# ccuchengwei/LongReadSelfCorrect

Measured on AMD Instinct MI355X. Metric: corrected Mbases/s (whole node), higher is better.
Workload: dtype int64

## Files before the change

longreadselfcorrect_amd/csrc/capi_correct.cpp:

```cpp
#include "capi_internal.h"

using namespace lrsc;

struct lrsc::CorrectScratch {
    DevBuf<ReadPlan> d_plan;
    DevBuf<uint32_t> d_pieces;
    DevBuf<uint8_t> d_codes_out;
    DevBuf<uint64_t> d_dst_off;
    DevBuf<char> d_dst;
    DevBuf<double> d_freqs;
    DpStage stage;
    DevBuf<WpReadWork> d_work;
    DevBuf<WpRead> d_reads;
    DevBuf<WpSlot> d_slots;
    DevBuf<uint64_t> d_sz;
    DevBuf<uint32_t> d_key, d_key_tmp, d_list, d_list_tmp;
    DevBuf<uint32_t> d_small;
    DevBuf<WpDpItem> d_items, d_items2, d_items3;
    DevBuf<DevCounters> d_ctr2;
    hipEvent_t ev_side_t0 = nullptr, ev_side_t1 = nullptr;
    DevBuf<WpRequest> d_req;
    DevBuf<uint8_t> d_prep, d_lane, d_lane_side, d_lane_wide;
    DevBuf<uint32_t> d_wide_list;
    DevBuf<uint32_t> d_sort9;
// ... 510 lines not shown
    for(unsigned m = 1; m < 34; ++m)
        if(hist[m]) std::fprintf(stderr, " %u:%.2f%%(%.1f%%)", m, 100.0 * hist[m] / n_range, 100.0 * wsteps[m] / std::max(tot, 1ull));
    const uint32_t qs[] = {n_range / 2, n_range / 10, n_range / 100, n_range / 1000, n_range / 10000};
    std::fprintf(stderr, "; leaf-steps at the median / top 10%% / 1%% / 0.1%% / 0.01%%: %u %u %u %u %u\n", hs[ord[qs[0]]].leaf_steps, hs[ord[qs[1]]].leaf_steps,
                 hs[ord[qs[2]]].leaf_steps, hs[ord[qs[3]]].leaf_steps, hs[ord[qs[4]]].leaf_steps);
    return LRSC_OK;
}

void WpFlow::print_round(const Round& R) const
{
    std::fprintf(stderr, "[lrsc] wp reads [%u, %u) round %u: %u entries, %u DP requests (%llu strings), arenas q %.1f MB prep %.1f MB path %.1f MB, %llu walks escalated so far\n",
                 r0, r1, R.index, R.n_ent, R.n_items, (unsigned long long)sc.stage.n_strings, R.tot[0] / 1048576.0, R.tot[1] / 1048576.0, R.tot[2] / 1048576.0,
                 (unsigned long long)n_escalated);
    const unsigned long long* g = R.begin_stats;
    if(tn.wp_begin_sort)
        std::fprintf(stderr, "[lrsc] wp reads [%u, %u) round %u: wp_begin %llu interval lists, %llu entries, every list sorted (LRSC_WP_BEGIN_SORT)\n",
                     r0, r1, R.index, g[0], g[2] + g[3]);
    else
        std::fprintf(stderr, "[lrsc] wp reads [%u, %u) round %u: wp_begin %llu interval lists, %llu with a repeated code (%.1f%%); entries %llu in the lists without one, %llu in those with one\n",
                     r0, r1, R.index, g[0], g[1], 100.0 * g[1] / std::max(g[0], 1ull), g[2], g[3]);
}

int WpFlow::print_extension_profile()
{
    unsigned long long prs[32];
    HIP_TRY(hipStreamSynchronize(ctx->stream));
    HIP_TRY(hipStreamSynchronize(sc.side));
    HIP_TRY(hipMemcpy(prs, sc.d_prof.p, sizeof(prs), hipMemcpyDeviceToHost));
    for(int part = 0; part < 2; ++part) {
        const unsigned long long* pr = prs + 16 * part;
        if(pr[10] == 0) continue;
        const double all = (double)pr[10], st = (double)std::max<unsigned long long>(pr[11], 1);
        std::fprintf(stderr, "[lrsc] wp extension kernel (%s), lane wall ticks: %.3g total, %.0f per step over %.3g steps; extendLeaves %.1f%% (refine %.1f%%, attempToExtend %.1f%% of which "
                             "getFMIndexExtensions %.1f%%), PrunedBySeedSupport %.1f%%, materialise+commit %.1f%%, isTerminated %.1f%%, refill %.1f%%, finish %.1f%%; single-leaf fast steps %.1f%% of the steps in %.1f%% of the ticks\n",
                     part ? "long-gap walks, one per wavefront" : "bulk and later rounds",
                     all, all / st, st, 100 * pr[0] / all, 100 * pr[1] / all, 100 * pr[2] / all, 100 * pr[3] / all, 100 * pr[4] / all, 100 * pr[5] / all, 100 * pr[6] / all,
                     100 * pr[8] / all, 100 * pr[9] / all, 100 * pr[12] / st, 100 * pr[7] / all);
    }
    return LRSC_OK;
}

int WpFlow::gather_results(lrsc_read_result* res, uint64_t* piece_off, uint64_t piece_cap, char* out, uint64_t out_cap,
                           uint64_t* n_pieces_out, uint64_t* out_used)
{
    std::vector<WpRead> ro(n);
    COPY_TRY(ctx, ro.data(), sc.d_reads.p, (size_t)n * sizeof(WpRead), hipMemcpyDeviceToHost);
    std::vector<uint32_t> pieces(std::max<uint64_t>(piece_total, 1));
    if(piece_total) COPY_TRY(ctx, pieces.data(), sc.d_pieces.p, (size_t)piece_total * sizeof(uint32_t), hipMemcpyDeviceToHost);
    std::vector<uint64_t> dst_off(n + 1, 0);
    uint64_t n_pieces = 0;
    for(uint32_t r = 0; r < n; ++r) {
        const WpRead& o = ro[r];
        int status = skipped[r];
        if(o.error == LRSC_WALK_ERR_GEOMETRY) status = LRSC_READ_GEOMETRY;
        else if(o.error == LRSC_WALK_ERR_CODE) status = LRSC_READ_INTERNAL;
        else if(o.error == LRSC_WALK_ERR_DP) status = LRSC_READ_DP_LIMIT;
        else if(o.error == LRSC_WALK_ERR_OUTPUT) status = LRSC_READ_OUTPUT_LIMIT;
        else if(o.error != 0) status = LRSC_READ_FRONTIER_LIMIT;
        lrsc_read_result& R = res[r];
        if(status != LRSC_READ_OK) {
            std::memset(&R, 0, sizeof(R));
            R.piece_first = n_pieces;
            R.status = status;
            dst_off[r + 1] = dst_off[r];
            continue;
        }
        R.merge = (int32_t)o.merge; R.n_pieces = o.n_pieces; R.piece_first = n_pieces;
        R.total_reads_len = (int64_t)(off[r + 1] - off[r]); R.corrected_len = o.c[1]; R.total_seed_num = seed_count[r]; R.total_walk_num = o.c[3];
        R.high_error_num = o.c[4]; R.exceed_depth_num = o.c[5]; R.exceed_leave_num = o.c[6]; R.fm_num = o.c[7];
// ... 64 lines not shown
```

longreadselfcorrect_amd/csrc/walk_device.h:

```cpp
#pragma once
#include <hip/hip_runtime.h>

#include "extend.h"
#include "introsort_emul.h"
#include "rank_device.h"

#ifndef LRSC_WALK_NOINLINE
#define LRSC_WALK_NOINLINE __noinline__
#endif
#ifndef LRSC_WALK_FN
#define LRSC_WALK_FN __device__
#endif

namespace lrsc {

constexpr uint64_t kNoKey = ~0ull;

template <bool WIDE>
LRSC_WALK_FN __forceinline__ void prepare_offset(const FmIndexDev& fm, const StrandC<typename Lay<WIDE>::pos_t>& sf,
                                               const StrandC<typename Lay<WIDE>::pos_t>& sr, const uint32_t* __restrict__ mtab,
                                               const uint8_t* __restrict__ q, uint32_t i, uint32_t Lq, uint32_t trg0,
                                               uint32_t seedk, uint32_t mink, SortItem* it9f, SortItem* it9r, uint8_t* flags5,
                                               typename Lay<WIDE>::pos_t* term, uint32_t& n_rank, uint32_t& n_blk)
{
    using P = typename Lay<WIDE>::pos_t;
    const bool want_term = i >= trg0 && i + mink <= Lq;
    uint32_t kmax = 0;
    if(i + 5 <= Lq) kmax = 5;
    if(i + seedk <= Lq) kmax = seedk;
    if(want_term) kmax = mink > kmax ? mink : kmax;
    WalkState<P> st = walk_init<P>();
    for(uint32_t s = 0; s < kmax;) {
        const uint32_t next_emit = s < 5 ? 5u : s < seedk ? seedk : mink;
        bool jumped = false;
        if(next_emit <= kmax) {
            WalkState<P> ts = walk_init<P>();
            const uint32_t tk = table_start<WIDE>(fm, [&](uint32_t t) { return (uint32_t)q[i + t]; }, next_emit, ts);
            if(tk == next_emit) { n_rank += st.n_rank; n_blk += st.n_blk; st = ts; st.n_rank = 0; st.n_blk = 0; s = tk; jumped = true; }
        }
        if(!jumped) { st = walk_step<WIDE>(sf, sr, q[i + s], 1u << 30, st, mtab); ++s; }
        if(st.size == 5) flags5[i] = (uint8_t)((st.fwd.lo <= st.fwd.hi ? 1 : 0) | (st.rvc.lo <= st.rvc.hi ? 2 : 0));
        if(st.size == seedk) {
            uint32_t code = 0;
            for(uint32_t t = 0; t < seedk; ++t) code = (code << 2) | q[i + t];
// ... 309 lines not shown
            const uint32_t back = U - 1 - t;
            return back < 32 ? (uint32_t)(slo >> (2 * back)) & 3u : (uint32_t)(shi >> (2 * (back - 32))) & 3u;
        };
        bool fb = false, rb = false;
        uint32_t t1 = 1;
        {
            WalkState<P> ts = walk_init<P>();
            const uint32_t tk = table_start<WIDE>(*fm, [&](uint32_t t) { return 3u - sc(U - 1 - t); }, Lw, ts);
            if(tk != 0) {
                f = ts.rvc; r = ts.fwd; fb = ts.rvc_broken; rb = ts.fwd_broken; t1 = tk;
            } else {
                f = init_interval<P>(sR, sc(U - 1));
                r = init_interval<P>(sF, 3u - sc(U - 1));
                n_rank += 2;
            }
        }
        for(uint32_t t = t1; t < Lw; ++t) {
            if(fb && rb) break;
            const uint32_t c = sc(U - 1 - t);
            if(!fb) { f = upd(sR, c, f); fb = f.lo > f.hi; }
            if(!rb) { r = upd(sF, 3u - c, r); rb = r.lo > r.hi; }
            if(fb && rb) break;
        }
    }
    LRSC_WALK_FN __forceinline__ void select_next(uint64_t slo, uint64_t shi, uint32_t U, uint32_t t, IvT<P>& f, IvT<P>& r)
    {
        const uint32_t back = U - 1 - t;
        const uint32_t b = back < 32 ? (uint32_t)(slo >> (2 * back)) & 3u : (uint32_t)(shi >> (2 * (back - 32))) & 3u;
        f = upd(sR, b, f);
        r = upd(sF, 3u - b, r);
    }
    LRSC_WALK_FN LRSC_WALK_NOINLINE uint64_t SelectFreqsOfrange(uint64_t LowerBound, uint64_t UpperBound, Leaf<P>* leaves, uint32_t n)
    {
        int tempmaxfmfreqs = 0;
        const uint32_t U = (uint32_t)UpperBound, Lw = (uint32_t)LowerBound;
        for(uint32_t j = 0; j < n; ++j) {
            Leaf<P>& lf = leaves[j];
            IvT<P> f, r;
            select_first(lf.suf_lo, lf.suf_hi, U, Lw, f, r);
            lf.tflo = f.lo; lf.tfhi = f.hi; lf.trlo = r.lo; lf.trhi = r.hi;
            lf.tmpFreq = (int)(isize(f.lo, f.hi) + isize(r.lo, r.hi));
            if(lf.tmpFreq > tempmaxfmfreqs) tempmaxfmfreqs = lf.tmpFreq;
        }
        if(tempmaxfmfreqs - (int)freqsOfKmerSize[LowerBound] < 5) return LowerBound;

        for(uint64_t i = 1; i <= UpperBound - LowerBound; i++) {
            tempmaxfmfreqs = 0;
            for(uint32_t j = 0; j < n; ++j) {
                Leaf<P>& lf = leaves[j];
                IvT<P> f{lf.tflo, lf.tfhi}, r{lf.trlo, lf.trhi};
                select_next(lf.suf_lo, lf.suf_hi, U, (uint32_t)(UpperBound - LowerBound - i), f, r);
                lf.tflo = f.lo; lf.tfhi = f.hi; lf.trlo = r.lo; lf.trhi = r.hi;
                lf.tmpFreq = (int)(isize(f.lo, f.hi) + isize(r.lo, r.hi));
                if(lf.tmpFreq > tempmaxfmfreqs) tempmaxfmfreqs = lf.tmpFreq;
            }
            if(tempmaxfmfreqs - (int)freqsOfKmerSize[LowerBound + i] < 5) return LowerBound + i;
        }
        return UpperBound;
    }
    LRSC_WALK_FN __forceinline__ uint64_t SelectFreqsOfrange1(uint64_t LowerBound, uint64_t UpperBound, uint64_t slo, uint64_t shi)
    {
        const uint32_t U = (uint32_t)UpperBound, Lw = (uint32_t)LowerBound;
        IvT<P> f, r;
        select_first(slo, shi, U, Lw, f, r);
        int freq = (int)(isize(f.lo, f.hi) + isize(r.lo, r.hi));
        int tempmaxfmfreqs = freq > 0 ? freq : 0;
// ... 96 lines not shown
    }

    LRSC_WALK_FN void attempToExtend()
    {
        double minimumErrorRate = 1;
        for(uint32_t i = 0; i < n_cur; i += 4) {
            double e[4];
#pragma unroll
            for(uint32_t j = 0; j < 4; ++j) e[j] = cur[i + j < n_cur ? i + j : i].localErr;
#pragma unroll
            for(uint32_t j = 0; j < 4; ++j) if(i + j < n_cur && e[j] < minimumErrorRate) minimumErrorRate = e[j];
        }
        uint32_t w = 0;
        for(uint32_t i = 0; i < n_cur; ++i) {
            const double errorRateDiff = cur[i].localErr - minimumErrorRate;
            if((errorRateDiff > 0.05 && currentLength > localK / 2) || (errorRateDiff > 0.1 && currentLength > 15)) {
                free_leaf_slots(cur[i]);
                continue;
            }
            if(w != i) leaf_move(&cur[w], &cur[i]);
            ++w;
        }
        n_cur = w;

        n_highfreq = 0;
        const int highfreqThreshold = PBcoverage > 60 ? (int)((uint64_t)(PBcoverage / 60) * 3) : 3;
        for(uint32_t i = 0; i < n_cur; ++i) {
            const Leaf<P> par = cur[i];
            Ext ext[4];
            uint32_t mask = 0;
            int count = 0;
            while(count < 2) {
                if(count == 1 && !(par.localErr == minimumErrorRate && n_cur > 1)) break;
                uint64_t tc;
                const uint64_t tg = tick();
                mask = getFMIndexExtensions_v(par.flo, par.fhi, par.rlo, par.rhi, par.tailLetterCount, par.suf_lo, ext, tc);
                tock(3, tg);
                if(mask != 0) break;
                min_SA_threshold--;
                count++;
            }
            min_SA_threshold += (uint64_t)count;
            if(mask == 0) continue;
            for(uint32_t b = 0; b < 4; ++b) {
                if(!(mask & (1u << b))) continue;
                if(n_nxt >= max_children()) { error = LRSC_WALK_ERR_CHILDREN; return; }
                const Leaf<P> ch = make_child(par, i, b, ext[b]);
                if(ch.kmerFrequency > highfreqThreshold) n_highfreq++;
                nxt[n_nxt++] = ch;
            }
        }
    }
    LRSC_WALK_FN __forceinline__ Leaf<P> make_child(const Leaf<P>& par, uint32_t i, uint32_t b, const Ext& e) const
    {
        Leaf<P> ch = par;
        ch.flo = e.f.lo; ch.fhi = e.f.hi; ch.rlo = e.r.lo; ch.rhi = e.r.hi;
        ch.kmerFrequency = e.freq;
        ch.currOverlapLen++;
        ch.queryOverlapLen++;
        if(par.tailLetter == b) ch.tailLetterCount = par.tailLetterCount + 1;
        else { ch.tailLetter = b; ch.tailLetterCount = 1; }
        suf_push(ch, b);
        ch.parent = (uint16_t)i;
        ch.ext = (uint8_t)b;
        ch.alive = 1;
        return ch;
    }

    LRSC_WALK_FN void extendLeaves()
    {
        n_nxt = 0;
        uint64_t t = tick();
        if(currentKmerSize > maxOverlap) refineSAInterval(cur, n_cur, maxOverlap);
        tock(1, t);
        t = tick();
        attempToExtend();
        tock(2, t);
        if(error) return;
        if(n_nxt == 0) {
            const uint64_t LowerBound = (currentKmerSize - 2) > minOverlap ? (currentKmerSize - 2) : minOverlap;
            const uint64_t ReduceSize = SelectFreqsOfrange(LowerBound, currentKmerSize, cur, n_cur);
            refineSAInterval(cur, n_cur, ReduceSize);
            attempToExtend();
            if(error) return;
            if(n_nxt == 0) {
                min_SA_threshold--;
                attempToExtend();
                min_SA_threshold++;
                if(error) return;
            }
        }
        if(n_nxt != 0) {
            currentLength++;
            currentKmerSize++;
            if(isInsufficientFreqs(n_highfreq, n_nxt)) {
                const uint64_t LowerBound = (currentKmerSize - 2) > minOverlap ? (currentKmerSize - 2) : minOverlap;
                const uint64_t ReduceSize = SelectFreqsOfrange(LowerBound, currentKmerSize, nxt, n_nxt);
                refineSAInterval(nxt, n_nxt, ReduceSize);
            }
        }
    }

    LRSC_WALK_FN LRSC_WALK_NOINLINE bool isSupportedByNewSeed(Leaf<P>& nd, uint64_t smallSeedIdx, uint64_t largeSeedIdx)
    {
        return seed_support_core(nd, smallSeedIdx, largeSeedIdx);
    }
    LRSC_WALK_FN __forceinline__ bool seed_support_core(Leaf<P>& nd, uint64_t smallSeedIdx, uint64_t largeSeedIdx)
    {
        const uint64_t seedIdxOffset = nd.lastOverlapLen < currentLength - seedSize ? (uint64_t)seedSize : currentLength - nd.lastOverlapLen;
        const uint64_t cand = nd.lastSeedIdx + seedIdxOffset;
        const uint64_t startSeedIdx = smallSeedIdx > cand ? smallSeedIdx : cand;
        bool isNewSeedFound = false;
        const bool fv = nd.flo <= nd.fhi, rv = nd.rlo <= nd.rhi;
        const uint32_t mask9 = seedSize >= 16 ? 0xFFFFFFFFu : ((1u << (2 * seedSize)) - 1u);
        const uint32_t code9 = (uint32_t)nd.suf_lo & mask9;
        const uint32_t hb = (code9 ^ (code9 >> 9)) & 255u;
        uint32_t jf = fv ? head9f[hb] : 0xFFFFu;
        uint32_t jr = rv ? head9r[hb] : 0xFFFFu;
        auto advance = [&](uint32_t j, const SortItem* it, const uint16_t* nx) -> uint32_t {
            while(j != 0xFFFFu && it[j].pad != code9) j = nx[j];
            return j;
        };
        jf = advance(jf, it9f, next9f);
        jr = advance(jr, it9r, next9r);
        int minIdxDiff = 10000;
        const uint64_t currSeedIdx = currentLength - seedSize;
        while(jf != 0xFFFFu || jr != 0xFFFFu) {
            const uint64_t vf = jf != 0xFFFFu ? it9f[jf].val : 0, vr = jr != 0xFFFFu ? it9r[jr].val : 0;
            if(fv && jf != 0xFFFFu && vf >= startSeedIdx && vf <= largeSeedIdx) {
                const int d = abs((int)vf - (int)currSeedIdx);
// ... 31 lines not shown
        double currErrorRate = unmatchedLen / totalLen;
        nd.globalErr = currErrorRate;
        const uint32_t totalsize = nd.hist_size + 1;
        nd.hist_size = totalsize;
        if(totalsize >= localK) {
            const double old = parent_ring[(totalsize - localK) % 100];
            currErrorRate = (currErrorRate * totalLen - old * (totalLen - localK)) / localK;
        }
        nd.localErr = currErrorRate;
        return currErrorRate;
    }

    template <bool INLINE>
    LRSC_WALK_FN __forceinline__ void prune_leaf(Leaf<P>& leaf, const double* pring, uint64_t currSeedIdx, uint64_t smallSeedIdx, uint64_t largeSeedIdx)
    {
        bool isNewSeedFound = false;
        if(currentLength - leaf.lastOverlapLen > seedSize || currentLength - leaf.lastOverlapLen <= 1) {
            const uint64_t preSeedIdx = leaf.lastSeedIdx;
            isNewSeedFound = INLINE ? seed_support_core(leaf, smallSeedIdx, largeSeedIdx) : isSupportedByNewSeed(leaf, smallSeedIdx, largeSeedIdx);
            if(isNewSeedFound) {
                if(currSeedIdx + (uint64_t)(int64_t)leaf.lastSeedIdxOffset - preSeedIdx > seedSize)
                    leaf.numRedeemSeed += (seedSize - 1) * PacBioErrorRate;
                leaf.lastSeedIdxOffset = (int)leaf.lastSeedIdx - (int)currSeedIdx;
            } else {
                const uint64_t v = currSeedIdx + (uint64_t)(int64_t)leaf.lastSeedIdxOffset - leaf.lastSeedIdx;
                if(v % seedSize == 1) leaf.numOfErrors++;
                else if(v > (uint64_t)seedSize - 1) leaf.numRedeemSeed += 1 - PacBioErrorRate;
            }
        } else
            leaf.numRedeemSeed += 1 - PacBioErrorRate;
        const double currErrorRate = computeErrorRate(leaf, pring);
        if(currErrorRate > errorRate) leaf.alive = 0;
    }
    LRSC_WALK_FN void PrunedBySeedSupport()
    {
        const uint64_t currSeedIdx = currentLength - seedSize;
        const uint64_t indelOffset = seedSize + maxIndelSize;
        const uint64_t smallSeedIdx = currSeedIdx <= indelOffset ? 0 : currSeedIdx - indelOffset;
        const uint64_t largeSeedIdx = (currSeedIdx + indelOffset) >= (Lq - seedSize) ? (Lq - seedSize) : currSeedIdx + indelOffset;
        alive_lo = 0; alive_hi = 0; has_child = 0;
        if constexpr(BIG) { bits_clear_all(this->alive_bits, n_nxt); bits_clear_all(this->child_bits, n_cur); }
        for(uint32_t c = 0; c < n_nxt; ++c) {
            Leaf<P> leaf = nxt[c];
            prune_leaf<true>(leaf, rings + (uint64_t)leaf.ring * 100, currSeedIdx, smallSeedIdx, largeSeedIdx);
            nxt[c] = leaf;
            if constexpr(BIG) { if(leaf.alive) { bits_set(this->alive_bits, c); bits_set(this->child_bits, leaf.parent); } }
            else if(leaf.alive) { if(c < 64) alive_lo |= 1ull << c; else alive_hi |= 1ull << (c - 64); has_child |= 1u << leaf.parent; }
        }
    }

    LRSC_WALK_FN LRSC_WALK_NOINLINE void terminated_leaf(Leaf<P>& lf, const uint32_t* pw, uint32_t plen, int extra)
    {
        const int hit = term_scan(lf);
        if(hit < 0) return;
        if(lf.res_first == -1) {
            if(n_results >= max_results()) { error = LRSC_WALK_ERR_RESULTS; return; }
            ++n_results;
            lf.res_first = (int)n_results;
        }
        lf.res_second = hit;
        term_store(lf, hit, pw, plen, extra);
    }
    LRSC_WALK_FN __forceinline__ int term_scan(const Leaf<P>& lf) const
    {
        const bool fvalid = lf.flo <= lf.fhi, rvalid = lf.rlo <= lf.rhi;
        if(currentKmerSize >= minOverlap) {
            const uint32_t L = minOverlap < 16 ? (uint32_t)minOverlap : 16u;
            const uint32_t code = (uint32_t)(lf.suf_lo & (L >= 16 ? 0xFFFFFFFFull : ((1ull << (2 * L)) - 1ull)));
            const uint32_t h = (code * 0x9E3779B1u) >> 25;
            if((((h < 64 ? tmask0 : tmask1) >> (h & 63u)) & 1ull) == 0) return -1;
        }
        const uint64_t i0 = (uint64_t)(lf.res_second > 0 ? lf.res_second : 0);
        int hit = -1;
        for(uint64_t i = i0; i <= (uint64_t)trg_len - (int)minOverlap; i++) {
            const P* t = term + i * 4;
            const bool isFwdTerminated = fvalid && lf.flo >= t[0] && lf.fhi <= t[1];
            const bool isRvcTerminated = rvalid && lf.rlo >= t[2] && lf.rhi <= t[3];
            if(isFwdTerminated || isRvcTerminated) hit = (int)i;
        }
        return hit;
    }
    LRSC_WALK_FN __forceinline__ void term_store(const Leaf<P>& lf, int hit, const uint32_t* pw, uint32_t plen, int extra)
    {
        WalkResultRec& r = results[lf.res_first - 1];
        r.error_rate = lf.globalErr;
        r.match_i = (uint32_t)hit;
        uint32_t* dst = rpaths + (uint64_t)(lf.res_first - 1) * pathw;
        const uint32_t nw = (plen + 15) >> 4;
        burst_copy4(dst, pw, nw);
        uint32_t len = plen;
        if(extra >= 0) { path_set(dst, len, (uint32_t)extra); ++len; }
        r.path_len = len;
    }

    LRSC_WALK_FN int run(uint32_t* out_len, uint32_t* out_words, uint32_t* out_match_i)
    {
        begin();
        while(step()) {}
        return finish(out_len, out_words, out_match_i);
    }

    bool ended;
    bool profile = false;
    bool escalate = false;
// ... 191 lines not shown
                const uint32_t Lm = minOverlap < 16 ? (uint32_t)minOverlap : 16u;
                const uint32_t code = (uint32_t)(L.suf_lo & (Lm >= 16 ? 0xFFFFFFFFull : ((1ull << (2 * Lm)) - 1ull)));
                const uint32_t h = (code * 0x9E3779B1u) >> 25;
                may_hit = (((h < 64 ? tmask0 : tmask1) >> (h & 63u)) & 1ull) != 0;
            }
            if(may_hit) {
                leave_fast(L);
                terminated_leaf(cur[0], paths + (uint64_t)L.path * pathw, L.path_len, -1);
                if(error) return 0;
                L.res_first = cur[0].res_first; L.res_second = cur[0].res_second;
            }
        }
        return 1;
    }

    LRSC_WALK_FN bool step()
    {
        if(ended || error || !(n_cur != 0 && n_cur <= maxLeaves && currentLength <= maxLength)) return false;
        leaf_steps += n_cur;
        if(n_cur > max_front) max_front = n_cur;
        if(profile) {
            const uint64_t t_step0 = __builtin_readcyclecounter();
            step_body();
            cyc_loop += __builtin_readcyclecounter() - t_step0;
        } else
            step_body();
        return true;
    }

    LRSC_WALK_FN void step_body()
    {
        {
            uint64_t t = tick();
            extendLeaves();
            tock(0, t);
            if(error) return;
            t = tick();
            PrunedBySeedSupport();
            tock(4, t);
            t = tick();
            uint32_t survivors = (uint32_t)(__builtin_popcountll(alive_lo) + __builtin_popcountll(alive_hi));
            if constexpr(BIG) { survivors = 0; for(uint32_t w = 0; w < bits_words(n_nxt); ++w) survivors += (uint32_t)__builtin_popcountll(this->alive_bits[w]); }
            auto is_alive = [&](uint32_t c) -> bool {
                if constexpr(BIG) return bits_get(this->alive_bits, c);
                else return ((c < 64 ? alive_lo >> c : alive_hi >> (c - 64)) & 1ull) != 0;
            };
            ++steps;
            if(survivors > maxLeaves) {
                if(currentLength >= minLength)
                    for(uint32_t c = 0; c < n_nxt; ++c) {
                        if(!is_alive(c)) continue;
                        const Leaf<P>& par = cur[nxt[c].parent];
                        terminated_leaf(nxt[c], paths + (uint64_t)par.path * pathw, par.path_len, (int)nxt[c].ext);
                        if(error) return;
                    }
                n_cur = survivors;
                ended = true;
                return;
            }
            if constexpr(BIG) { for(uint32_t i = 0; i < n_cur; ++i) if(!bits_get(this->child_bits, i)) free_leaf_slots(cur[i]); }
            else for(uint32_t i = 0; i < n_cur; ++i) if(!((has_child >> i) & 1u)) free_leaf_slots(cur[i]);
            const bool want_term = currentLength >= minLength;
            uint32_t seen = 0, w = 0;
            if constexpr(BIG) bits_clear_all(this->seen_bits, n_cur);
            for(uint32_t c = 0; c < n_nxt; ++c) {
                if(!is_alive(c)) continue;
                Leaf<P> ch = nxt[c];
                bool further;
                if constexpr(BIG) further = bits_get(this->seen_bits, ch.parent); else further = ((seen >> ch.parent) & 1u) != 0;
                if(further) {
                    const uint16_t pr = ch.ring, pp = ch.path;
                    if constexpr(BIG) {
                        ch.ring = (uint16_t)bits_take_lowest(this->ring_bits, this->cap);
                        ch.path = (uint16_t)bits_take_lowest(this->path_bits, this->cap);
                    } else {
                        ch.ring = (uint16_t)__builtin_ctz(ring_free); ring_free &= ring_free - 1u;
                        ch.path = (uint16_t)__builtin_ctz(path_free); path_free &= path_free - 1u;
                    }
                    const uint32_t live = ch.hist_size - 1 < 100 ? ch.hist_size - 1 : 100;
                    const uint32_t nburst = (live * 8 + kCopyChunk16 * 16 - 1) / (kCopyChunk16 * 16);
                    burst_copy16(rings + (uint64_t)ch.ring * 100, rings + (uint64_t)pr * 100, nburst);
                    burst_copy4(paths + (uint64_t)ch.path * pathw, paths + (uint64_t)pp * pathw, (ch.path_len + 16) >> 4);
                }
                if constexpr(BIG) bits_set(this->seen_bits, ch.parent); else seen |= 1u << ch.parent;
                rings[(uint64_t)ch.ring * 100 + (ch.hist_size - 1) % 100] = ch.globalErr;
                path_set(paths + (uint64_t)ch.path * pathw, ch.path_len, ch.ext);
                ch.path_len++;
                nxt[w] = ch;
                ++w;
            }
            (void)want_term;
            if(4u * w <= (cur == leaf_small ? small_cap() : max_children())) { Leaf<P>* t2 = cur; cur = nxt; nxt = t2; }
            else for(uint32_t i = 0; i < w; ++i) leaf_move(&cur[i], &nxt[i]);
            n_cur = w;
            tock(5, t);
            t = tick();
            if(currentLength >= minLength)
                for(uint32_t i = 0; i < n_cur; ++i) {
                    terminated_leaf(cur[i], paths + (uint64_t)cur[i].path * pathw, cur[i].path_len, -1);
                    if(error) return;
                }
            tock(6, t);
        }
    }

    LRSC_WALK_FN LRSC_WALK_NOINLINE int finish(uint32_t* out_len, uint32_t* out_words, uint32_t* out_match_i)
    {
        if(escalate && (ended || error == LRSC_WALK_ERR_RESULTS)) return LRSC_WALK_NEEDS_WIDE;
        if(error) return error;
        if(n_results > 0) {
            double minErrorRate = 1;
            int best = -1;
            for(uint32_t i = 0; i < n_results; ++i)
                if(results[i].error_rate < minErrorRate) { minErrorRate = results[i].error_rate; best = (int)i; }
            if(best < 0) return -4;
            *out_len = results[best].path_len;
            *out_match_i = results[best].match_i;
            const uint32_t* src = rpaths + (uint64_t)best * pathw;
            const uint32_t nw = (results[best].path_len + 15) >> 4;
            burst_copy4(out_words, src, nw);
            return 1;
        }
        if(n_cur == 0) return -1;
        else if(currentLength > maxLength) return -2;
        else if(n_cur > maxLeaves) return -3;
        return -4;
    }
};

template <bool WIDE, bool BIG>
__device__ __forceinline__ void walk_bind_work(Walk<WIDE, BIG>& W, const FmIndexDev& fm, const uint32_t* mtab, const ExtendArgs& a,
                                               const WalkWork& ww, uint8_t* ws)
{
// ... 28 lines not shown
```

longreadselfcorrect_amd/csrc/wp.hip:

```cpp
#define LRSC_WALK_FN __device__ __forceinline__
#define LRSC_WALK_NOINLINE
#include <hip/hip_runtime.h>
#include <hipcub/hipcub.hpp>

#include <algorithm>

#include "walk_device.h"
#include "wp.h"
#include "wp_walk.h"

namespace lrsc {

constexpr uint64_t kWpBeginSortBlocks = 32768;

#ifndef LRSC_WP_EXTEND_OCC
#define LRSC_WP_EXTEND_OCC 2
#endif

struct WpGeom {
    int k, interval, trg_len, T_start, T_len;
    bool rtou, bad;
    uint32_t lq, pathw;
};
__device__ __forceinline__ WpGeom wp_geometry(const WpArgs& a, int S_seedLen, int S_end, int S_endBest, bool S_isRepeat, const int32_t* T)
// ... 260 lines not shown
        Walk<false>::sort9(reinterpret_cast<SortItem*>(ws + (r ? L.item9r : L.item9f)), r ? H->n9r : H->n9f,
                           reinterpret_cast<uint16_t*>(ws + L.head9) + 256u * r, reinterpret_cast<uint16_t*>(ws + (r ? L.next9r : L.next9f)));
    }
}

template <bool WIDE>
__global__ __launch_bounds__(64, LRSC_WP_EXTEND_OCC) void wp_extend_kernel(FmIndexDev fm, WpArgs a)
{
    using P = typename Lay<WIDE>::pos_t;
    __shared__ __attribute__((aligned(16))) uint32_t mtab[MaskTabSize<WIDE>::value];
    init_mask_table<WIDE>(mtab);
    const uint32_t stride = a.lane_stride ? a.lane_stride : 1u;
    const bool owner = (threadIdx.x % stride) == 0;
    const uint32_t lane_id = owner ? (blockIdx.x * 64 + threadIdx.x) / stride : 0xFFFFFFFFu;
    Walk<WIDE> W;
    wp_walk_consts(W, fm, a, mtab);
    const WpLaneLayout LL = wp_lane_layout(a.lbytes, a.lane_pathw);
    uint8_t* lws = a.lane_ws + (uint64_t)(owner ? lane_id : 0u) * a.lane_ws_bytes;
    Leaf<P>* const leaf_base = reinterpret_cast<Leaf<P>*>(lws + LL.leaves);
    W.rings = reinterpret_cast<double*>(lws + LL.rings);
    W.results = reinterpret_cast<WalkResultRec*>(lws + LL.results);
    W.paths = reinterpret_cast<uint32_t*>(lws + LL.paths);
    W.pathw = a.lane_pathw;
    W.rpaths = W.paths + (uint64_t)32 * a.lane_pathw;

    bool in_walk = false;
    uint32_t si = 0;
    uint64_t steps0 = 0;
    Leaf<P> L;
    uint32_t pw = 0;
    bool fast = false;
    uint32_t gen_wait = 0;
    bool want_gen = false;
    uint64_t pr[8] = {0, 0, 0, 0, 0, 0, 0, 0};
    uint64_t t_refill = 0, t_finish = 0, n_fast = 0;
    const bool prof = a.prof != nullptr;
    if(prof) W.prof = pr;
    const uint64_t t_loop0 = prof ? __builtin_readcyclecounter() : 0;
    if(lane_id < a.n_lanes)
    while(true) {
        if(!in_walk) {
            const uint64_t tr0 = prof ? __builtin_readcyclecounter() : 0;
            const uint32_t i = atomicAdd(a.queue, 1u);
            if(i >= a.n_list) break;
            if(a.reqs && a.reqs[i].kind != kWpReqFm) continue;
            si = a.list ? a.list[i] : (uint32_t)a.slot_base + i;
            const WpSlot& s = a.slots[si];
            if(s.flags & kWpGeomBad) continue;
            W.cur = leaf_base; W.nxt = leaf_base + 32; W.leaf_small = leaf_base;
            steps0 = W.steps;
            wp_walk_bind(W, a, s);
            in_walk = true;
            fast = false; want_gen = false; gen_wait = 0;
            if(prof) t_refill += __builtin_readcyclecounter() - tr0;
        }
        if(!fast && !want_gen && W.can_fast()) { W.enter_fast(L, pw); fast = true; }
        int r = 2;
        if(fast) {
            const uint64_t tq = prof ? __builtin_readcyclecounter() : 0;
            r = W.step_fast(L, pw);
            if(r != 1) fast = false;
            if(prof) { pr[7] += __builtin_readcyclecounter() - tq; if(r == 1) ++n_fast; }
        }
        const uint32_t n_fast_now = (uint32_t)__builtin_popcountll(__ballot(r == 1));
        if(r == 2) {
            const uint32_t n_need = (uint32_t)__builtin_popcountll(__ballot(true));
            const uint32_t n_busy = n_need + n_fast_now;
            const bool waited = __ballot(gen_wait >= a.general_max_wait) != 0;
            if(n_need * 100u < n_busy * a.general_quorum_pct && !waited) { ++gen_wait; want_gen = true; continue; }
            gen_wait = 0; want_gen = false;
            r = W.step() ? 1 : 0;
        }
        if(r == 1) continue;
        in_walk = false;
        const uint64_t tf0 = prof ? __builtin_readcyclecounter() : 0;
        wp_walk_finish(W, a, si, steps0);
        if(prof) t_finish += __builtin_readcyclecounter() - tf0;
    }
    if(prof && lane_id < a.n_lanes) {
        for(int j = 0; j < 8; ++j) atomicAdd(&a.prof[j], (unsigned long long)pr[j]);
        atomicAdd(&a.prof[8], (unsigned long long)t_refill);
        atomicAdd(&a.prof[9], (unsigned long long)t_finish);
        atomicAdd(&a.prof[10], (unsigned long long)(__builtin_readcyclecounter() - t_loop0));
        atomicAdd(&a.prof[11], (unsigned long long)W.steps);
        atomicAdd(&a.prof[12], (unsigned long long)n_fast);
    }
    flush_counters(a.ctr, W.n_rank, W.n_blk);
}

__global__ __launch_bounds__(256) void wp_dp_collect_kernel(WpArgs a, const WpDpItem* items)
{
    const uint32_t i = blockIdx.x * 256 + threadIdx.x;
    if(i >= a.n_dp) return;
    WpSlot& s = a.slots[items[i].slot];
    const DpMsaOut m = a.dp_msa[i];
    s.dp_rows = m.n_rows; s.dp_cons_len = m.cons_len; s.dp_error = m.error;
    s.dp_cons = a.dp_cons + a.dp_reqs[i].cons_off;
    s.flags |= (uint8_t)kWpDpValid;
}

__global__ __launch_bounds__(64) void wp_stitch_kernel(WpArgs a)
{
    const uint32_t r = a.r0 + blockIdx.x, lane = threadIdx.x;
    const WpReadWork rw = a.work[r];
    WpRead& R = a.reads[r];
    if(R.started && R.state == kReadDone) return;
    const uint64_t rs = a.read_off[r];
    const uint32_t rlen = (uint32_t)(a.read_off[r + 1] - rs);
    const uint8_t* read = a.codes + rs;
    const uint32_t n_seeds = rw.n_seeds;
    const int32_t* seeds = a.seeds + seed_slab(rs, r, a.min_k) * kSeedInts;
    uint8_t* out = a.out_codes + rw.out_off;
    uint8_t* wl = a.walk_log ? a.walk_log + seed_slab(rs, r, a.min_k) : nullptr;
    uint32_t* piece_start = a.piece_start + rw.piece_off;

    int64_t correctedLen = 0, totalWalkNum = 0, highErrorNum = 0, exceedDepthNum = 0, exceedLeaveNum = 0, FMNum = 0, DPNum = 0, seedDis = 0;
    uint64_t steps = 0;
    uint32_t out_len = 0, n_pieces = 0, it = 1;
// ... 294 lines not shown
```

Baseline: 149.0.

## Batch seed-support pruning, commit, and terminal scan in small leaf groups

PrunedBySeedSupport now handles leaves in pairs. Their fields are loaded up front and the two hash-chain searches are walked in lockstep, so independent memory loads can overlap. The commit loop also works in groups of two with batched field and path-word loads, and the termination loop prefilters leaves with a cheap hash-mask check in groups of four before calling terminated_leaf. Profiling gains a SelectFreqsOfrange timer and no-op trace hooks, at the cost of more register pressure and more complex control flow.

```diff
diff --git a/longreadselfcorrect_amd/csrc/capi_correct.cpp b/longreadselfcorrect_amd/csrc/capi_correct.cpp
--- a/longreadselfcorrect_amd/csrc/capi_correct.cpp
+++ b/longreadselfcorrect_amd/csrc/capi_correct.cpp
@@ -566,9 +566,9 @@
         if(pr[10] == 0) continue;
         const double all = (double)pr[10], st = (double)std::max<unsigned long long>(pr[11], 1);
         std::fprintf(stderr, "[lrsc] wp extension kernel (%s), lane wall ticks: %.3g total, %.0f per step over %.3g steps; extendLeaves %.1f%% (refine %.1f%%, attempToExtend %.1f%% of which "
-                             "getFMIndexExtensions %.1f%%), PrunedBySeedSupport %.1f%%, materialise+commit %.1f%%, isTerminated %.1f%%, refill %.1f%%, finish %.1f%%; single-leaf fast steps %.1f%% of the steps in %.1f%% of the ticks\n",
+                             "getFMIndexExtensions %.1f%%; SelectFreqsOfrange %.1f%%), PrunedBySeedSupport %.1f%%, materialise+commit %.1f%%, isTerminated %.1f%%, refill %.1f%%, finish %.1f%%; single-leaf fast steps %.1f%% of the steps in %.1f%% of the ticks\n",
                      part ? "long-gap walks, one per wavefront" : "bulk and later rounds",
-                     all, all / st, st, 100 * pr[0] / all, 100 * pr[1] / all, 100 * pr[2] / all, 100 * pr[3] / all, 100 * pr[4] / all, 100 * pr[5] / all, 100 * pr[6] / all,
+                     all, all / st, st, 100 * pr[0] / all, 100 * pr[1] / all, 100 * pr[2] / all, 100 * pr[3] / all, 100 * pr[13] / all, 100 * pr[4] / all, 100 * pr[5] / all, 100 * pr[6] / all,
                      100 * pr[8] / all, 100 * pr[9] / all, 100 * pr[12] / st, 100 * pr[7] / all);
     }
     return LRSC_OK;
diff --git a/longreadselfcorrect_amd/csrc/walk_device.h b/longreadselfcorrect_amd/csrc/walk_device.h
--- a/longreadselfcorrect_amd/csrc/walk_device.h
+++ b/longreadselfcorrect_amd/csrc/walk_device.h
@@ -10,6 +10,9 @@
 #endif
 #ifndef LRSC_WALK_FN
 #define LRSC_WALK_FN __device__
+#endif
+#ifndef LRSC_WALK_TRACE
+#define LRSC_WALK_TRACE(kind, a, b)
 #endif
 
 namespace lrsc {
@@ -385,6 +388,7 @@
     }
     LRSC_WALK_FN LRSC_WALK_NOINLINE uint64_t SelectFreqsOfrange(uint64_t LowerBound, uint64_t UpperBound, Leaf<P>* leaves, uint32_t n)
     {
+        LRSC_WALK_TRACE(3, n, 0);
         int tempmaxfmfreqs = 0;
         const uint32_t U = (uint32_t)UpperBound, Lw = (uint32_t)LowerBound;
         for(uint32_t j = 0; j < n; ++j) {
@@ -547,6 +551,7 @@
             int count = 0;
             while(count < 2) {
                 if(count == 1 && !(par.localErr == minimumErrorRate && n_cur > 1)) break;
+                if(count == 1) { LRSC_WALK_TRACE(2, i, n_cur); }
                 uint64_t tc;
                 const uint64_t tg = tick();
                 mask = getFMIndexExtensions_v(par.flo, par.fhi, par.rlo, par.rhi, par.tailLetterCount, par.suf_lo, ext, tc);
@@ -559,7 +564,7 @@
             if(mask == 0) continue;
             for(uint32_t b = 0; b < 4; ++b) {
                 if(!(mask & (1u << b))) continue;
-                if(n_nxt >= max_children()) { error = LRSC_WALK_ERR_CHILDREN; return; }
+                if(n_nxt >= max_children()) { LRSC_WALK_TRACE(4, n_nxt, i); error = LRSC_WALK_ERR_CHILDREN; return; }
                 const Leaf<P> ch = make_child(par, i, b, ext[b]);
                 if(ch.kmerFrequency > highfreqThreshold) n_highfreq++;
                 nxt[n_nxt++] = ch;
@@ -594,7 +599,9 @@
         if(error) return;
         if(n_nxt == 0) {
             const uint64_t LowerBound = (currentKmerSize - 2) > minOverlap ? (currentKmerSize - 2) : minOverlap;
+            const uint64_t ts = tick();
             const uint64_t ReduceSize = SelectFreqsOfrange(LowerBound, currentKmerSize, cur, n_cur);
+            tock(8, ts);
             refineSAInterval(cur, n_cur, ReduceSize);
             attempToExtend();
             if(error) return;
@@ -610,7 +617,9 @@
             currentKmerSize++;
             if(isInsufficientFreqs(n_highfreq, n_nxt)) {
                 const uint64_t LowerBound = (currentKmerSize - 2) > minOverlap ? (currentKmerSize - 2) : minOverlap;
+                const uint64_t ts = tick();
                 const uint64_t ReduceSize = SelectFreqsOfrange(LowerBound, currentKmerSize, nxt, n_nxt);
+                tock(8, ts);
                 refineSAInterval(nxt, n_nxt, ReduceSize);
             }
         }
@@ -708,6 +717,9 @@
         const double currErrorRate = computeErrorRate(leaf, pring);
         if(currErrorRate > errorRate) leaf.alive = 0;
     }
+    static constexpr uint32_t kPruneGroup = 2;
+    static constexpr uint32_t kCommitGroup = 2;
+    static constexpr uint32_t kTermGroup = 4;
     LRSC_WALK_FN void PrunedBySeedSupport()
     {
         const uint64_t currSeedIdx = currentLength - seedSize;
@@ -716,12 +728,128 @@
         const uint64_t largeSeedIdx = (currSeedIdx + indelOffset) >= (Lq - seedSize) ? (Lq - seedSize) : currSeedIdx + indelOffset;
         alive_lo = 0; alive_hi = 0; has_child = 0;
         if constexpr(BIG) { bits_clear_all(this->alive_bits, n_nxt); bits_clear_all(this->child_bits, n_cur); }
-        for(uint32_t c = 0; c < n_nxt; ++c) {
-            Leaf<P> leaf = nxt[c];
-            prune_leaf<true>(leaf, rings + (uint64_t)leaf.ring * 100, currSeedIdx, smallSeedIdx, largeSeedIdx);
-            nxt[c] = leaf;
-            if constexpr(BIG) { if(leaf.alive) { bits_set(this->alive_bits, c); bits_set(this->child_bits, leaf.parent); } }
-            else if(leaf.alive) { if(c < 64) alive_lo |= 1ull << c; else alive_hi |= 1ull << (c - 64); has_child |= 1u << leaf.parent; }
+        constexpr uint32_t G = kPruneGroup;
+        constexpr uint32_t NIL = 0xFFFFu;
+        const uint32_t mask9 = seedSize >= 16 ? 0xFFFFFFFFu : ((1u << (2 * seedSize)) - 1u);
+        for(uint32_t c0 = 0; c0 < n_nxt; c0 += G) {
+            const uint32_t g = n_nxt - c0 < G ? n_nxt - c0 : G;
+            uint64_t lastSeedIdx[G], lastOverlapLen[G], totalSeeds[G], currOverlapLen[G], numOfErrors[G], queryOverlapLen[G];
+            double numRedeemSeed[G];
+            uint32_t hist_size[G], code9[G], ring[G], parent[G];
+            int32_t lastSeedIdxOffset[G];
+            bool fv[G], rv[G];
+#pragma unroll
+            for(uint32_t j = 0; j < G; ++j) {
+                const Leaf<P>& lf = nxt[c0 + (j < g ? j : 0)];
+                lastSeedIdx[j] = lf.lastSeedIdx; lastOverlapLen[j] = lf.lastOverlapLen; totalSeeds[j] = lf.totalSeeds;
+                currOverlapLen[j] = lf.currOverlapLen; numOfErrors[j] = lf.numOfErrors; queryOverlapLen[j] = lf.queryOverlapLen;
+                numRedeemSeed[j] = lf.numRedeemSeed; hist_size[j] = lf.hist_size; lastSeedIdxOffset[j] = lf.lastSeedIdxOffset;
+                code9[j] = (uint32_t)lf.suf_lo & mask9; ring[j] = lf.ring; parent[j] = lf.parent;
+                fv[j] = lf.flo <= lf.fhi; rv[j] = lf.rlo <= lf.rhi;
+            }
+            bool need[G];
+            uint64_t preSeedIdx[G], startSeedIdx[G];
+            uint32_t jf[G], jr[G];
+            double old[G];
+#pragma unroll
+            for(uint32_t j = 0; j < G; ++j) {
+                const uint64_t d = currentLength - lastOverlapLen[j];
+                need[j] = j < g && (d > seedSize || d <= 1);
+                preSeedIdx[j] = lastSeedIdx[j];
+                const uint64_t seedIdxOffset = lastOverlapLen[j] < currentLength - seedSize ? (uint64_t)seedSize : currentLength - lastOverlapLen[j];
+                const uint64_t cand = lastSeedIdx[j] + seedIdxOffset;
+                startSeedIdx[j] = smallSeedIdx > cand ? smallSeedIdx : cand;
+                const uint32_t hb = (code9[j] ^ (code9[j] >> 9)) & 255u;
+                jf[j] = head9f[hb]; jr[j] = head9r[hb];
+                const uint32_t totalsize = hist_size[j] + 1;
+                old[j] = rings[(uint64_t)ring[j] * 100 + (totalsize >= localK ? (totalsize - localK) % 100 : 0)];
+            }
+            bool mf[G], mr[G], found[G];
+            uint32_t vf[G], vr[G];
+            int minIdxDiff[G];
+#pragma unroll
+            for(uint32_t j = 0; j < G; ++j) {
+                if(!(need[j] && fv[j])) jf[j] = NIL;
+                if(!(need[j] && rv[j])) jr[j] = NIL;
+                mf[j] = false; mr[j] = false; found[j] = false; vf[j] = 0; vr[j] = 0; minIdxDiff[j] = 10000;
+            }
+            while(true) {
+                bool seek = false;
+#pragma unroll
+                for(uint32_t j = 0; j < G; ++j) seek = seek || (!mf[j] && jf[j] != NIL) || (!mr[j] && jr[j] != NIL);
+                if(seek) {
+                    uint32_t pf[G], pr_[G], wf[G], wr[G], nf[G], nr[G];
+#pragma unroll
+                    for(uint32_t j = 0; j < G; ++j) {
+                        const uint32_t a = (!mf[j] && jf[j] != NIL) ? jf[j] : 0u, b = (!mr[j] && jr[j] != NIL) ? jr[j] : 0u;
+                        pf[j] = it9f[a].pad; wf[j] = it9f[a].val; nf[j] = next9f[a];
+                        pr_[j] = it9r[b].pad; wr[j] = it9r[b].val; nr[j] = next9r[b];
+                    }
+#pragma unroll
+                    for(uint32_t j = 0; j < G; ++j) {
+                        if(!mf[j] && jf[j] != NIL) { if(pf[j] == code9[j]) { mf[j] = true; vf[j] = wf[j]; } jf[j] = nf[j]; }
+                        if(!mr[j] && jr[j] != NIL) { if(pr_[j] == code9[j]) { mr[j] = true; vr[j] = wr[j]; } jr[j] = nr[j]; }
+                    }
+                    continue;
+                }
+                bool any = false;
+#pragma unroll
+                for(uint32_t j = 0; j < G; ++j) {
+                    if(!(mf[j] || mr[j])) continue;
+                    any = true;
+                    const uint64_t f = vf[j], r = vr[j];
+                    if(mf[j] && f >= startSeedIdx[j] && f <= largeSeedIdx) {
+                        const int d = abs((int)f - (int)currSeedIdx);
+                        if(d < minIdxDiff[j]) { lastSeedIdx[j] = f; queryOverlapLen[j] = f + seedSize; minIdxDiff[j] = d; }
+                        lastOverlapLen[j] = currentLength;
+                        currOverlapLen[j] = currentLength;
+                        found[j] = true;
+                    } else if(mr[j] && r >= startSeedIdx[j] && r <= largeSeedIdx) {
+                        const int d = abs((int)currSeedIdx - (int)r);
+                        if(d < minIdxDiff[j]) { lastSeedIdx[j] = r; queryOverlapLen[j] = r + seedSize; minIdxDiff[j] = d; }
+                        lastOverlapLen[j] = currentLength;
+                        currOverlapLen[j] = currentLength;
+                        found[j] = true;
+                    }
+                    mf[j] = false; mr[j] = false;
+                }
+                if(!any) break;
+            }
+#pragma unroll
+            for(uint32_t j = 0; j < G; ++j) {
+                if(j >= g) continue;
+                const uint32_t c = c0 + j;
+                if(need[j]) {
+                    if(found[j]) {
+                        totalSeeds[j]++;
+                        if(currSeedIdx + (uint64_t)(int64_t)lastSeedIdxOffset[j] - preSeedIdx[j] > seedSize)
+                            numRedeemSeed[j] += (seedSize - 1) * PacBioErrorRate;
+                        lastSeedIdxOffset[j] = (int)lastSeedIdx[j] - (int)currSeedIdx;
+                    } else {
+                        const uint64_t v = currSeedIdx + (uint64_t)(int64_t)lastSeedIdxOffset[j] - lastSeedIdx[j];
+                        if(v % seedSize == 1) numOfErrors[j]++;
+                        else if(v > (uint64_t)seedSize - 1) numRedeemSeed[j] += 1 - PacBioErrorRate;
+                    }
+                } else
+                    numRedeemSeed[j] += 1 - PacBioErrorRate;
+                double matchedLen = (double)totalSeeds[j] + seedSize - 1;
+                matchedLen += numRedeemSeed[j];
+                const double totalLen = (double)currOverlapLen[j];
+                const double unmatchedLen = totalLen - matchedLen;
+                double currErrorRate = unmatchedLen / totalLen;
+                const double globalErr = currErrorRate;
+                const uint32_t totalsize = hist_size[j] + 1;
+                if(totalsize >= localK) currErrorRate = (currErrorRate * totalLen - old[j] * (totalLen - localK)) / localK;
+                const bool alive = !(currErrorRate > errorRate);
+                Leaf<P>& lf = nxt[c];
+                lf.lastSeedIdx = lastSeedIdx[j]; lf.lastOverlapLen = lastOverlapLen[j]; lf.totalSeeds = totalSeeds[j];
+                lf.currOverlapLen = currOverlapLen[j]; lf.numOfErrors = numOfErrors[j]; lf.queryOverlapLen = queryOverlapLen[j];
+                lf.numRedeemSeed = numRedeemSeed[j]; lf.localErr = currErrorRate; lf.globalErr = globalErr;
+                lf.hist_size = totalsize; lf.lastSeedIdxOffset = lastSeedIdxOffset[j];
+                if(!alive) lf.alive = 0;
+                if constexpr(BIG) { if(alive) { bits_set(this->alive_bits, c); bits_set(this->child_bits, parent[j]); } }
+                else if(alive) { if(c < 64) alive_lo |= 1ull << c; else alive_hi |= 1ull << (c - 64); has_child |= 1u << parent[j]; }
+            }
         }
     }
 
@@ -737,15 +865,20 @@
         lf.res_second = hit;
         term_store(lf, hit, pw, plen, extra);
     }
-    LRSC_WALK_FN __forceinline__ int term_scan(const Leaf<P>& lf) const
-    {
-        const bool fvalid = lf.flo <= lf.fhi, rvalid = lf.rlo <= lf.rhi;
+    LRSC_WALK_FN __forceinline__ bool term_may_hit(uint64_t suf_lo) const
+    {
         if(currentKmerSize >= minOverlap) {
             const uint32_t L = minOverlap < 16 ? (uint32_t)minOverlap : 16u;
-            const uint32_t code = (uint32_t)(lf.suf_lo & (L >= 16 ? 0xFFFFFFFFull : ((1ull << (2 * L)) - 1ull)));
+            const uint32_t code = (uint32_t)(suf_lo & (L >= 16 ? 0xFFFFFFFFull : ((1ull << (2 * L)) - 1ull)));
             const uint32_t h = (code * 0x9E3779B1u) >> 25;
-            if((((h < 64 ? tmask0 : tmask1) >> (h & 63u)) & 1ull) == 0) return -1;
-        }
+            if((((h < 64 ? tmask0 : tmask1) >> (h & 63u)) & 1ull) == 0) return false;
+        }
+        return true;
+    }
+    LRSC_WALK_FN __forceinline__ int term_scan(const Leaf<P>& lf) const
+    {
+        const bool fvalid = lf.flo <= lf.fhi, rvalid = lf.rlo <= lf.rhi;
+        if(!term_may_hit(lf.suf_lo)) return -1;
         const uint64_t i0 = (uint64_t)(lf.res_second > 0 ? lf.res_second : 0);
         int hit = -1;
         for(uint64_t i = i0; i <= (uint64_t)trg_len - (int)minOverlap; i++) {
@@ -1003,9 +1136,11 @@
     {
         {
             uint64_t t = tick();
+            LRSC_WALK_TRACE(0, n_cur, 0);
             extendLeaves();
             tock(0, t);
             if(error) return;
+            LRSC_WALK_TRACE(1, n_nxt, 0);
             t = tick();
             PrunedBySeedSupport();
             tock(4, t);
@@ -1031,45 +1166,75 @@
             }
             if constexpr(BIG) { for(uint32_t i = 0; i < n_cur; ++i) if(!bits_get(this->child_bits, i)) free_leaf_slots(cur[i]); }
             else for(uint32_t i = 0; i < n_cur; ++i) if(!((has_child >> i) & 1u)) free_leaf_slots(cur[i]);
-            const bool want_term = currentLength >= minLength;
+            constexpr uint32_t G = kCommitGroup;
             uint32_t seen = 0, w = 0;
             if constexpr(BIG) bits_clear_all(this->seen_bits, n_cur);
-            for(uint32_t c = 0; c < n_nxt; ++c) {
-                if(!is_alive(c)) continue;
-                Leaf<P> ch = nxt[c];
-                bool further;
-                if constexpr(BIG) further = bits_get(this->seen_bits, ch.parent); else further = ((seen >> ch.parent) & 1u) != 0;
-                if(further) {
-                    const uint16_t pr = ch.ring, pp = ch.path;
-                    if constexpr(BIG) {
-                        ch.ring = (uint16_t)bits_take_lowest(this->ring_bits, this->cap);
-                        ch.path = (uint16_t)bits_take_lowest(this->path_bits, this->cap);
-                    } else {
-                        ch.ring = (uint16_t)__builtin_ctz(ring_free); ring_free &= ring_free - 1u;
-                        ch.path = (uint16_t)__builtin_ctz(path_free); path_free &= path_free - 1u;
+            for(uint32_t c0 = 0; c0 < n_nxt; c0 += G) {
+                bool live[G];
+                uint32_t parent[G], ring[G], path[G], hist_size[G], plen[G], ext[G];
+                double globalErr[G];
+                bool anylive = false;
+#pragma unroll
+                for(uint32_t j = 0; j < G; ++j) { live[j] = c0 + j < n_nxt && is_alive(c0 + j); anylive = anylive || live[j]; }
+                if(!anylive) continue;
+#pragma unroll
+                for(uint32_t j = 0; j < G; ++j) {
+                    const Leaf<P>& lf = nxt[live[j] ? c0 + j : c0];
+                    parent[j] = lf.parent; ring[j] = lf.ring; path[j] = lf.path; hist_size[j] = lf.hist_size; plen[j] = lf.path_len;
+                    ext[j] = lf.ext; globalErr[j] = lf.globalErr;
+                }
+#pragma unroll
+                for(uint32_t j = 0; j < G; ++j) {
+                    if(!live[j]) continue;
+                    bool further;
+                    if constexpr(BIG) further = bits_get(this->seen_bits, parent[j]); else further = ((seen >> parent[j]) & 1u) != 0;
+                    if(further) {
+                        const uint32_t pr = ring[j], pp = path[j];
+                        if constexpr(BIG) {
+                            ring[j] = bits_take_lowest(this->ring_bits, this->cap);
+                            path[j] = bits_take_lowest(this->path_bits, this->cap);
+                        } else {
+                            ring[j] = (uint32_t)__builtin_ctz(ring_free); ring_free &= ring_free - 1u;
+                            path[j] = (uint32_t)__builtin_ctz(path_free); path_free &= path_free - 1u;
+                        }
+                        const uint32_t nlive = hist_size[j] - 1 < 100 ? hist_size[j] - 1 : 100;
+                        const uint32_t nburst = (nlive * 8 + kCopyChunk16 * 16 - 1) / (kCopyChunk16 * 16);
+                        burst_copy16(rings + (uint64_t)ring[j] * 100, rings + (uint64_t)pr * 100, nburst);
+                        burst_copy4(paths + (uint64_t)path[j] * pathw, paths + (uint64_t)pp * pathw, (plen[j] + 16) >> 4);
                     }
-                    const uint32_t live = ch.hist_size - 1 < 100 ? ch.hist_size - 1 : 100;
-                    const uint32_t nburst = (live * 8 + kCopyChunk16 * 16 - 1) / (kCopyChunk16 * 16);
-                    burst_copy16(rings + (uint64_t)ch.ring * 100, rings + (uint64_t)pr * 100, nburst);
-                    burst_copy4(paths + (uint64_t)ch.path * pathw, paths + (uint64_t)pp * pathw, (ch.path_len + 16) >> 4);
+                    if constexpr(BIG) bits_set(this->seen_bits, parent[j]); else seen |= 1u << parent[j];
                 }
-                if constexpr(BIG) bits_set(this->seen_bits, ch.parent); else seen |= 1u << ch.parent;
-                rings[(uint64_t)ch.ring * 100 + (ch.hist_size - 1) % 100] = ch.globalErr;
-                path_set(paths + (uint64_t)ch.path * pathw, ch.path_len, ch.ext);
-                ch.path_len++;
-                nxt[w] = ch;
-                ++w;
-            }
-            (void)want_term;
+                uint32_t word[G];
+#pragma unroll
+                for(uint32_t j = 0; j < G; ++j) word[j] = paths[(uint64_t)path[j] * pathw + (plen[j] >> 4)];
+#pragma unroll
+                for(uint32_t j = 0; j < G; ++j) {
+                    if(!live[j]) continue;
+                    rings[(uint64_t)ring[j] * 100 + (hist_size[j] - 1) % 100] = globalErr[j];
+                    const uint32_t sh = 2 * (plen[j] & 15u);
+                    paths[(uint64_t)path[j] * pathw + (plen[j] >> 4)] = (word[j] & ~(3u << sh)) | (ext[j] << sh);
+                    if(w != c0 + j) leaf_move(&nxt[w], &nxt[c0 + j]);
+                    nxt[w].ring = (uint16_t)ring[j]; nxt[w].path = (uint16_t)path[j]; nxt[w].path_len = plen[j] + 1;
+                    ++w;
+                }
+            }
             if(4u * w <= (cur == leaf_small ? small_cap() : max_children())) { Leaf<P>* t2 = cur; cur = nxt; nxt = t2; }
             else for(uint32_t i = 0; i < w; ++i) leaf_move(&cur[i], &nxt[i]);
             n_cur = w;
             tock(5, t);
             t = tick();
             if(currentLength >= minLength)
-                for(uint32_t i = 0; i < n_cur; ++i) {
-                    terminated_leaf(cur[i], paths + (uint64_t)cur[i].path * pathw, cur[i].path_len, -1);
-                    if(error) return;
+                for(uint32_t i0 = 0; i0 < n_cur; i0 += kTermGroup) {
+                    uint64_t slo[kTermGroup];
+#pragma unroll
+                    for(uint32_t j = 0; j < kTermGroup; ++j) slo[j] = cur[i0 + j < n_cur ? i0 + j : i0].suf_lo;
+#pragma unroll
+                    for(uint32_t j = 0; j < kTermGroup; ++j) {
+                        const uint32_t i = i0 + j;
+                        if(i >= n_cur || !term_may_hit(slo[j])) continue;
+                        terminated_leaf(cur[i], paths + (uint64_t)cur[i].path * pathw, cur[i].path_len, -1);
+                        if(error) return;
+                    }
                 }
             tock(6, t);
         }
diff --git a/longreadselfcorrect_amd/csrc/wp.hip b/longreadselfcorrect_amd/csrc/wp.hip
--- a/longreadselfcorrect_amd/csrc/wp.hip
+++ b/longreadselfcorrect_amd/csrc/wp.hip
@@ -316,7 +316,7 @@
     bool fast = false;
     uint32_t gen_wait = 0;
     bool want_gen = false;
-    uint64_t pr[8] = {0, 0, 0, 0, 0, 0, 0, 0};
+    uint64_t pr[9] = {0, 0, 0, 0, 0, 0, 0, 0, 0};
     uint64_t t_refill = 0, t_finish = 0, n_fast = 0;
     const bool prof = a.prof != nullptr;
     if(prof) W.prof = pr;
@@ -368,6 +368,7 @@
         atomicAdd(&a.prof[10], (unsigned long long)(__builtin_readcyclecounter() - t_loop0));
         atomicAdd(&a.prof[11], (unsigned long long)W.steps);
         atomicAdd(&a.prof[12], (unsigned long long)n_fast);
+        atomicAdd(&a.prof[13], (unsigned long long)pr[8]);
     }
     flush_counters(a.ctr, W.n_rank, W.n_blk);
 }
```

After: 157.6, median of 6. 5.8% higher.
